# mlefkir/Pioran.jl

Hardware: AMD Instinct MI355X
Metric: logpdf evals/sec (batched) at N=1e4, J=20; max |Δlogℒ| vs reference (higher is better)
Workload: dtype f64; 1 GPU; N=10000 irregular series, SHO-20 (J=20 celerite terms, R=40 active rows), batch=4096 draws per GPU, shared (c,d), per-draw mu/nu; inputs HBM-resident; N=10000, J=20, R_active=40, batch_per_gpu=4096, global_batch=4096, kernel_config=tile, parallelism=batch-sharded x1, all-gather of logL

## Files before the change

pioran.jl_amd/csrc/celerite_tile.hip:

```cpp
#include "common.h"
#include "window_common.h"

#ifndef PIORAN_TSTAMP
#define PIORAN_TSTAMP(i) __builtin_amdgcn_sched_barrier(0)
#define PIORAN_TSTAMP_DECL
#define PIORAN_TSTAMP_FLUSH
#endif
#ifndef PIORAN_ASTAMP2
#define PIORAN_ASTAMP2(i) __builtin_amdgcn_sched_barrier(0)
#define PIORAN_ASTAMP2_DECL
#define PIORAN_ASTAMP2_FLUSH
#endif

namespace {

constexpr int kTileMaxTerms = 64;
constexpr int kTileWaves = 4;
#define PIORAN_LDS_ORDER() asm volatile("" ::: "memory")
template <int NB, bool CD = false>
constexpr int tile_adj_waves() { return NB <= 3 ? 4 : (CD ? 2 : 3); }

template <int NB>
struct TileWave {
    double scr[16 * 18];
    double2 albe[16 * NB];
    double ck[16 * NB + 16];
    double ys[16];
    double up[NB > 1 ? NB * (NB - 1) / 2 : 1][16 * 18];
};

constexpr int kPairWin = 5;
template <int JQ>
__global__ void __launch_bounds__(256) tile_pairs_mfma_kernel(const ScanParams p, const double* __restrict__ btab, int64_t rsb, int64_t tsp, double* __restrict__ out)
{
    const int J = p.J;
    const int64_t NW = (p.N + KW - 1) / KW;
    const int lane = threadIdx.x & 63, w = threadIdx.x >> 6, li = lane & 15, lk = lane >> 4;
    const int64_t b0 = ((int64_t)blockIdx.y * 4 + w) * 16;
    if (b0 >= p.B) return;
    const int64_t draw = b0 + li < p.B ? b0 + li : p.B - 1;
    double aop[JQ], bop[JQ];
    int toff[JQ];
#pragma unroll
    for (int q = 0; q < JQ; ++q) {
        const int t = 4 * q + lk;
        aop[q] = t < J ? p.A[draw * J + t] : 0.0;
        bop[q] = t < J ? p.Bc[draw * J + t] : 0.0;
        toff[q] = (t < J ? t : J - 1) * 128 + 4 * (li & 3) + (li >> 2);
    }
    const bool live = b0 + li < p.B;
    double* orow = out + (b0 + li) * NW * 128 + 4 * lk;
    const int64_t k0 = (int64_t)blockIdx.x * kPairWin, k1 = k0 + kPairWin < NW ? k0 + kPairWin : NW;
    for (int64_t k = k0; k < k1; ++k) {
        const double2* E = reinterpret_cast<const double2*>(btab + k * rsb + tsp);
#pragma unroll 2
        for (int pt = 0; pt < 8; ++pt) {
            double2 e[JQ];
#pragma unroll
            for (int q = 0; q < JQ; ++q) e[q] = E[toff[q] + 16 * pt];
            d4 acc = {0.0, 0.0, 0.0, 0.0};
#pragma unroll
            for (int q = 0; q < JQ; ++q) {
                acc = __builtin_amdgcn_mfma_f64_16x16x4f64(e[q].x, aop[q], acc, 0, 0, 0);
                acc = __builtin_amdgcn_mfma_f64_16x16x4f64(e[q].y, bop[q], acc, 0, 0, 0);
            }
            if (live) *reinterpret_cast<d4*>(orow + k * 128 + 16 * pt) = acc;
        }
    }
}

template <typename... Args>
static inline bool launch_pairs_mfma(const ScanParams& p, hipStream_t stream, Args... args)
{
    const int64_t NW = (p.N + KW - 1) / KW;
    if ((p.B + 63) / 64 > 65535 || p.J > kTileMaxTerms) return false;
    const dim3 gr((unsigned)((NW + kPairWin - 1) / kPairWin), (unsigned)((p.B + 63) / 64));
    const int jq = (p.J + 3) / 4;
    if (jq <= 5) hipLaunchKernelGGL(tile_pairs_mfma_kernel<5>, gr, dim3(256), 0, stream, p, args...);
    else if (jq <= 10) hipLaunchKernelGGL(tile_pairs_mfma_kernel<10>, gr, dim3(256), 0, stream, p, args...);
    else if (jq <= 16) hipLaunchKernelGGL(tile_pairs_mfma_kernel<16>, gr, dim3(256), 0, stream, p, args...);
    else return false;
    return true;
}

template <int NB, int KL = 4, bool ST = false, bool SER = false>
__global__ void __launch_bounds__(64 * kTileWaves, NB <= 4 ? 2 : 1) celerite_tile_kernel(const ScanParams p, const double* __restrict__ btab,
                                                                                          const double* __restrict__ pairs)
{
    constexpr int TS = 3 * NB * 256 + 16 * NB + 16, TSP = (TS + 127) & ~127;
    static_assert(!(ST && SER), "the gradient's forward pass takes the shared series only");
    extern __shared__ double lds_[];
    const int tid = threadIdx.x;
    const int w = __builtin_amdgcn_readfirstlane(tid >> 6);
    const int lane = tid & 63, q = lane >> 4, c16 = lane & 15;
    const int64_t b = (int64_t)blockIdx.x * kTileWaves + w;
    if (b >= p.B) return;
    const int64_t N = p.N;
    const int J = p.J, R = p.R;
    const int64_t NW = (N + KW - 1) / KW;
    const int64_t RSB = TSP + 256 * (int64_t)J;
    TileWave<NB>& sw = reinterpret_cast<TileWave<NB>*>(lds_)[w];
    const __amdgpu_buffer_rsrc_t rs_tab = __builtin_amdgcn_make_buffer_rsrc(const_cast<double*>(btab), 0, 0x7ffffffc, 0x00020000);
    const __amdgpu_buffer_rsrc_t rs_pw = __builtin_amdgcn_make_buffer_rsrc(const_cast<double*>(pairs + b * NW * 128), 0, 0x7ffffffc, 0x00020000);
    const int lane8 = lane * 8;
    const int rsb8 = (int)(RSB * 8);
    constexpr int Jy = NB - 1;
    const int ry = R & 15;
    const double mu = p.mu ? p.mu[b] : 0.0;
    const double nu = p.nu ? p.nu[b] : 1.0;
    const bool has_nu = p.nu != nullptr;
    const double* __restrict__ Ab_ = p.A + b * J;
    const double* __restrict__ Bb_ = p.Bc + b * J;
    double suma = 0.0;
    for (int j = 0; j < J; ++j) suma += Ab_[j];

    for (int r = lane; r < 16 * NB; r += 64) {
        double a = 0.0, bb = 0.0;
        if (r < R) {
            const int rm = p.rowmap[r];
            const int term = rm & 0xfffff;
            a = Ab_[term];
            bb = ((rm >> 30) & 1) ? -Bb_[term] : Bb_[term];
        }
        sw.albe[r] = double2{a, bb};
    }
    constexpr int NU = NB * (NB - 1) / 2;
    for (int i = lane; i < (NU > 0 ? NU : 1) * 16 * 18; i += 64) (&sw.up[0][0])[i] = 0.0;
    asm volatile("s_waitcnt lgkmcnt(0)" ::: "memory");

    constexpr int NT = NB * (NB + 1) / 2;
    auto tix = [](int I, int Jc) constexpr { return I * (I + 1) / 2 + Jc; };
    auto uix = [](int I, int Jc) constexpr { return I * (I - 1) / 2 + Jc; };
    d4 T[NT];
#pragma unroll
    for (int i = 0; i < NT; ++i) T[i] = d4{0.0, 0.0, 0.0, 0.0};
    double Uf[NB][4];

    double cvn[4], cxn[4];
    auto live_k = [](int I, int ks) constexpr { return I < NB - 1 || ks < KL; };
    auto fetch_u = [&](int64_t k, int I) __attribute__((always_inline)) {
        const int so = (int)k * rsb8;
#pragma unroll
        for (int ks = 0; ks < 4; ++ks) {
            if (!live_k(I, ks)) continue;
            cvn[ks] = buf_load_f64(rs_tab, lane8, so + (I * 4 + ks) * 512);
            cxn[ks] = buf_load_f64(rs_tab, lane8, so + (NB * 256 + (I * 4 + ks) * 64) * 8);
        }
    };
    auto form_u = [&](int I) __attribute__((always_inline)) {
        if (I == NB - 1 && KL == 0) return;
        double2 cf[4];
#pragma unroll
        for (int ks = 0; ks < 4; ++ks)
            if (live_k(I, ks)) cf[ks] = sw.albe[16 * I + 4 * ks + q];
        asm volatile("s_waitcnt lgkmcnt(0)" ::: "memory");
#pragma unroll
        for (int ks = 0; ks < 4; ++ks)
            if (live_k(I, ks)) Uf[I][ks] = fma(cf[ks].x, cvn[ks], cf[ks].y * cxn[ks]);
    };
    constexpr int NCK = (16 * NB + 16 + 63) / 64;
    double ckpre[NCK];
    auto fetch_ck = [&](int64_t k) __attribute__((always_inline)) {
        const int so = (int)k * rsb8 + 3 * NB * 256 * 8;
#pragma unroll
        for (int i = 0; i < NCK; ++i) ckpre[i] = buf_load_f64(rs_tab, lane8, so + 512 * i);
    };
    int pidx[4];
#pragma unroll
    for (int g = 0; g < 4; ++g) {
        const int r = 4 * g + q, hi = r > c16 ? r : c16, lo = r > c16 ? c16 : r;
        pidx[g] = 8 * (r == c16 ? 127 : hi * (hi - 1) / 2 + lo);
    }
    const int gd = (c16 - q) >> 2;
    const bool on_diag = ((c16 - q) & 3) == 0;
    double apre[4];
    auto fetch_A = [&](int64_t k) __attribute__((always_inline)) {
#pragma unroll
        for (int g = 0; g < 4; ++g) apre[g] = buf_load_f64(rs_pw, pidx[g], (int)k * 1024);
    };
    [[maybe_unused]] double ypre = 0.0, spre = 0.0;
    auto fetch_series = [&](int64_t k) __attribute__((always_inline)) {
        if constexpr (SER) {
            int64_t n = k * KW + c16;
            n = n < N ? n : N - 1;
            ypre = p.Y[b * N + n];
            spre = p.S2[b * N + n];
        }
    };
    fetch_A(0);
    fetch_ck(0);
    fetch_series(0);
#pragma unroll
    for (int I = 0; I < NB; ++I) {
        fetch_u(0, I);
        form_u(I);
    }
    const double mu_y = c16 == ry ? mu : 0.0;
    const int64_t k_ragged = (N % KW) ? NW - 1 : NW;
    double quad = 0.0;
    double Pm = 1.0;
    int Pe = 0;
    bool nonpd = false;

    PIORAN_TSTAMP_DECL
    for (int64_t k = 0; k < NW; ++k) {
        PIORAN_TSTAMP(0);
        const int wso = (int)k * rsb8;
        const bool more = k + 1 < NW;
#pragma unroll
        for (int i = 0; i < NCK; ++i)
            if (lane + 64 * i < 16 * NB + 16) sw.ck[lane + 64 * i] = ckpre[i];
        if constexpr (SER) {
            asm volatile("s_waitcnt lgkmcnt(0)" ::: "memory");
            if (lane < 16) { sw.ys[lane] = ypre; sw.ck[16 * NB + lane] = spre; }
        }
        if (more) { fetch_ck(k + 1); fetch_series(k + 1); }
        if constexpr (ST) {
            d4* gtk = reinterpret_cast<d4*>(p.gw + ((b * NW + k) * NT) * 256);
#pragma unroll
            for (int i = 0; i < NT; ++i) gtk[i * 64 + lane] = T[i];
        }
        constexpr bool VHA = NB <= 3 || NB >= 5;
        [[maybe_unused]] double vha[VHA ? NB : 1][4];
        if constexpr (VHA) {
#pragma unroll
            for (int I = 0; I < NB; ++I)
#pragma unroll
                for (int g = 0; g < 4; ++g) vha[I][g] = buf_load_f64(rs_tab, lane8, wso + (2 * NB * 256 + (I * 4 + g) * 64) * 8);
            if (k == k_ragged) {
#pragma unroll
                for (int I = 0; I < NB; ++I)
#pragma unroll
                    for (int g = 0; g < 4; ++g)
                        if (k * KW + 4 * g + q >= N) vha[I][g] = I == Jy ? mu_y : 0.0;
            }
        }
        d4 x[NB];
#pragma unroll
        for (int Jc = 0; Jc < NB; ++Jc) {
            d4 acc = {0.0, 0.0, 0.0, 0.0};
#pragma unroll
            for (int I = 0; I < Jc; ++I) {
                double bt[4];
#pragma unroll
                for (int ks = 0; ks < 4; ++ks) bt[ks] = sw.up[uix(Jc, I)][c16 * 18 + 4 * ks + q];
#pragma unroll
                for (int ks = 0; ks < 4; ++ks) acc = __builtin_amdgcn_mfma_f64_16x16x4f64(Uf[I][ks], bt[ks], acc, 0, 0, 0);
            }
#pragma unroll
            for (int I = Jc; I < NB; ++I)
#pragma unroll
                for (int ks = 0; ks < 4; ++ks)
                    if (live_k(I, ks)) acc = __builtin_amdgcn_mfma_f64_16x16x4f64(Uf[I][ks], T[tix(I, Jc)][ks], acc, 0, 0, 0);
            x[Jc] = acc;
        }
        PIORAN_TSTAMP(1);
        d4 G = {0.0, 0.0, 0.0, 0.0};
        double vh[4];
        if constexpr (!VHA) {
#pragma unroll
            for (int g = 0; g < 4; ++g) vh[g] = buf_load_f64(rs_tab, lane8, wso + (2 * NB * 256 + g * 64) * 8);
        }
        [[maybe_unused]] double ysv[4] = {0.0, 0.0, 0.0, 0.0};
        if constexpr (SER) {
#pragma unroll
            for (int g = 0; g < 4; ++g) ysv[g] = sw.ys[4 * g + q];
        }
#pragma unroll
        for (int Jc = 0; Jc < NB; ++Jc) {
            const bool gk = Jc < NB - 1 || KL > 0;
            if (gk) {
#pragma unroll
                for (int g = 0; g < 4; ++g) sw.scr[(4 * g + q) * 18 + c16] = x[Jc][g];
            }
            PIORAN_LDS_ORDER();
            double mb[4];
#pragma unroll
            for (int ks = 0; ks < 4; ++ks)
                if (live_k(Jc, ks)) mb[ks] = sw.scr[c16 * 18 + 4 * ks + q];
            const double ckc = sw.ck[16 * Jc + c16];
            asm volatile("s_waitcnt lgkmcnt(0)" ::: "memory");
#pragma unroll
            for (int ks = 0; ks < 4; ++ks)
                if (live_k(Jc, ks)) G = __builtin_amdgcn_mfma_f64_16x16x4f64(Uf[Jc][ks], mb[ks], G, 0, 0, 0);
#pragma unroll
            for (int g = 0; g < 4; ++g) {
                double v;
                if constexpr (VHA) v = vha[Jc][g]; else v = vh[g];
                if (Jc == Jy) v -= mu_y;
                x[Jc][g] = fma(-ckc, x[Jc][g], v);
                asm volatile("" : "+v"(x[Jc][g]));
            }
            if constexpr (!VHA) {
                if (Jc + 1 < NB) {
#pragma unroll
                    for (int g = 0; g < 4; ++g) vh[g] = buf_load_f64(rs_tab, lane8, wso + (2 * NB * 256 + ((Jc + 1) * 4 + g) * 64) * 8);
                }
            }
            __builtin_amdgcn_sched_barrier(0);
        }
        if constexpr (!VHA) {
            if (k == k_ragged) {
#pragma unroll
                for (int Jc = 0; Jc < NB; ++Jc)
#pragma unroll
                    for (int g = 0; g < 4; ++g) {
                        const double vt = buf_load_f64(rs_tab, lane8, wso + (2 * NB * 256 + (Jc * 4 + g) * 64) * 8);
                        if (k * KW + 4 * g + q >= N) x[Jc][g] -= Jc == Jy ? vt - mu_y : vt;
                    }
            }
        }
        if constexpr (SER) {
#pragma unroll
            for (int g = 0; g < 4; ++g) {
                double vt;
                if constexpr (VHA) vt = vha[Jy][g]; else vt = buf_load_f64(rs_tab, lane8, wso + (2 * NB * 256 + (Jy * 4 + g) * 64) * 8);
                const bool pad = k == k_ragged && k * KW + 4 * g + q >= N;
                if (c16 == ry && !pad) x[Jy][g] += ysv[g] - vt;
            }
        }
        PIORAN_TSTAMP(2);
        PIORAN_TSTAMP(3);
        {
            const double s2n = sw.ck[16 * NB + c16];
            const double dg = k * KW + c16 < N ? suma + (has_nu ? nu * s2n : s2n) : 1.0;
#pragma unroll
            for (int g = 0; g < 4; ++g) sw.scr[(4 * g + q) * 16 + c16] = ((on_diag && g == gd) ? dg : apre[g]) - G[g];
        }
        if (k + 1 < NW) fetch_A(k + 1);
        PIORAN_LDS_ORDER();
        double m[16];
#pragma unroll
        for (int j = 0; j < 16; ++j) m[j] = sw.scr[j * 16 + c16];
        asm volatile("s_waitcnt lgkmcnt(0)" ::: "memory");
        PIORAN_TSTAMP(4);
        __builtin_amdgcn_s_setprio(2);
        double mult = ldl_first_mult(m, c16);
        static_for<0, 16>([&](auto Pc) __attribute__((always_inline)) { ldl_step<decltype(Pc)::value>(m, mult, c16); });
        __builtin_amdgcn_s_setprio(0);
        PIORAN_TSTAMP(5);
        if (q == 0) {
            double2* dst = reinterpret_cast<double2*>(sw.scr + c16 * 18);
#pragma unroll
            for (int j = 0; j < 16; j += 2) dst[j / 2] = double2{m[j], m[j + 1]};
        }
        PIORAN_LDS_ORDER();
        double li[4], idv[4];
#pragma unroll
        for (int ks = 0; ks < 4; ++ks) {
            const int kk = 4 * ks + q;
            const double lv = sw.scr[kk * 18 + c16];
            idv[ks] = recip_f64(sw.scr[kk * 18 + kk]);
            li[ks] = kk < c16 ? lv * idv[ks] : (kk == c16 ? 1.0 : 0.0);
        }
        {
            const double dj = sw.scr[c16 * 18 + c16];
            nonpd |= !(dj > 0.0);
            Pm *= (k == 0 && c16 == 0) ? dj : fabs(dj);
            int ex;
            Pm = frexp(Pm, &ex);
            Pe += ex;
        }
        asm volatile("s_waitcnt lgkmcnt(0)" ::: "memory");
        PIORAN_TSTAMP(6);
        if (more) fetch_u(k + 1, 0);
        __builtin_amdgcn_sched_barrier(0);
        d4 yt[NB];
#pragma unroll
        for (int Jc = 0; Jc < NB; ++Jc) {
            d4 a = {0.0, 0.0, 0.0, 0.0};
#pragma unroll
            for (int ks = 0; ks < 4; ++ks) a = __builtin_amdgcn_mfma_f64_16x16x4f64(li[ks], x[Jc][ks], a, 0, 0, 0);
            yt[Jc] = a;
        }
        PIORAN_TSTAMP(7);
        constexpr bool CKP = NB <= 3 || NB >= 5;
        [[maybe_unused]] double ckrow[CKP ? NB : 1][4], ckcol[CKP ? NB : 1];
        if constexpr (CKP) {
#pragma unroll
            for (int I = 0; I < NB; ++I) {
#pragma unroll
                for (int g = 0; g < 4; ++g) ckrow[I][g] = sw.ck[16 * I + 4 * g + q];
                ckcol[I] = sw.ck[16 * I + c16];
            }
        }
        auto ck_row = [&](int I, int g) __attribute__((always_inline)) -> double { if constexpr (CKP) return ckrow[I][g]; else return sw.ck[16 * I + 4 * g + q]; };
#pragma unroll
        for (int Jc = 0; Jc < NB; ++Jc) {
            if (more) {
                form_u(Jc);
                if (Jc + 1 < NB) fetch_u(k + 1, Jc + 1);
            }
            double ysc[4];
            double ckc;
            if constexpr (CKP) ckc = ckcol[Jc]; else ckc = sw.ck[16 * Jc + c16];
#pragma unroll
            for (int g = 0; g < 4; ++g) {
                ysc[g] = yt[Jc][g] * idv[g];
                if (Jc == Jy) quad = fma(yt[Jc][g], ysc[g], quad);
            }
#pragma unroll
            for (int I = Jc; I < NB; ++I) {
#pragma unroll
                for (int g = 0; g < 4; ++g) T[tix(I, Jc)][g] *= ck_row(I, g) * ckc;
#pragma unroll
                for (int ks = 0; ks < 4; ++ks) T[tix(I, Jc)] = __builtin_amdgcn_mfma_f64_16x16x4f64(yt[I][ks], ysc[ks], T[tix(I, Jc)], 0, 0, 0);
                if (Jc < I) {
#pragma unroll
                    for (int g = 0; g < 4; ++g) sw.up[uix(I, Jc)][(4 * g + q) * 18 + c16] = T[tix(I, Jc)][g];
                }
            }
            __builtin_amdgcn_sched_barrier(0);
        }
        PIORAN_TSTAMP(8);
        PIORAN_LDS_ORDER();
    }

    PIORAN_TSTAMP_FLUSH
    asm volatile("s_waitcnt lgkmcnt(0)" ::: "memory");
    if (c16 == ry) sw.scr[q] = quad;
    if (q == 0) sw.scr[16 + c16] = log(Pm) + (double)Pe * 0.6931471805599453094;
    const bool any_nonpd = __builtin_amdgcn_ballot_w64(nonpd) != 0;
    asm volatile("s_waitcnt lgkmcnt(0)" ::: "memory");
    if (lane == 0) {
        const double qs = (sw.scr[0] + sw.scr[1]) + (sw.scr[2] + sw.scr[3]);
        double logdet = 0.0;
        for (int j = 0; j < 16; ++j) logdet += sw.scr[16 + j];
        const double res = -0.5 * logdet - 0.5 * (double)N * 1.8378770664093454836 - 0.5 * qs;
        p.out[b] = res;
        if (p.status) p.status[b] = !isfinite(res) ? 2 : (any_nonpd ? 1 : 0);
    }
}

template <int NB, bool CD = false>
struct TileAdjWave {
    double scr[16 * 18];
    double srm[16 * 16];
    double2 albe[16 * NB];
    double ck[16 * NB + 16];
    double qy[16];
    double red[16 * NB][4];
    double tk[NB * (NB + 1) / 2][16 * 18];
    double upB[NB > 1 ? NB * (NB - 1) / 2 : 1][16 * 18];
    double mw[CD ? NB : 1][CD ? 256 : 1];
    double accd[CD ? 2 * NB : 1][CD ? 64 : 1];
    double tm[CD ? 24 : 1];
    double scrb[(NB <= 3 && !CD) ? NB : 1][(NB <= 3 && !CD) ? 16 * 18 : 1];
    double acab[2 * NB][64];
};

template <int NB, bool CD>
constexpr bool tile_adj_batched() { return NB <= 3 && !CD; }
template <int NB, bool CD = false>
__global__ void __launch_bounds__((64 * tile_adj_waves<NB, CD>()), 1) celerite_tile_adjoint_kernel(const ScanParams p, const double* __restrict__ btab,
                                                                                                  const double* __restrict__ gtab, double* __restrict__ pairs,
                                                                                                  double* __restrict__ grad_a, double* __restrict__ grad_b,
                                                                                                  double* __restrict__ grad_nu, double* __restrict__ grad_mu,
                                                                                                  double* __restrict__ grad_c, double* __restrict__ grad_d)
{
    constexpr int TS = 3 * NB * 256 + 16 * NB + 16, TSP = (TS + 127) & ~127;
    constexpr int64_t GS = 4 * (int64_t)NB * 256 + 16 * NB + 16 + 24;
    constexpr int NT = NB * (NB + 1) / 2, NU = NB * (NB - 1) / 2;
    constexpr bool BT = tile_adj_batched<NB, CD>();
    extern __shared__ double lds_[];
    const int tid = threadIdx.x;
    const int w = __builtin_amdgcn_readfirstlane(tid >> 6);
    const int lane = tid & 63, q = lane >> 4, c16 = lane & 15;
    const int64_t b = (int64_t)blockIdx.x * tile_adj_waves<NB, CD>() + w;
    if (b >= p.B) return;
    const int64_t N = p.N;
    const int J = p.J, R = p.R;
    const int64_t NW = (N + KW - 1) / KW;
    const int64_t RSB = TSP + 256 * (int64_t)J;
    TileAdjWave<NB, CD>& sw = reinterpret_cast<TileAdjWave<NB, CD>*>(lds_)[w];
    const __amdgpu_buffer_rsrc_t rs_tab = __builtin_amdgcn_make_buffer_rsrc(const_cast<double*>(btab), 0, 0x7ffffffc, 0x00020000);
    const __amdgpu_buffer_rsrc_t rs_gt = __builtin_amdgcn_make_buffer_rsrc(const_cast<double*>(gtab), 0, 0x7ffffffc, 0x00020000);
    double* const pw = pairs + b * NW * 128;
    const double* const gtb = p.gw + b * NW * NT * 256;
    const int lane8 = lane * 8;
    const int rsb8 = (int)(RSB * 8), gs8 = (int)(GS * 8);
    constexpr int Jy = NB - 1;
    const int ry = R & 15;
    const double mu = p.mu ? p.mu[b] : 0.0;
    const double nu = p.nu ? p.nu[b] : 1.0;
    const bool has_nu = p.nu != nullptr;
    const double* __restrict__ Ab_ = p.A + b * J;
    const double* __restrict__ Bb_ = p.Bc + b * J;
    double suma = 0.0;
    for (int j = 0; j < J; ++j) suma += Ab_[j];
    for (int r = lane; r < 16 * NB; r += 64) {
        double a = 0.0, bb = 0.0;
        if (r < R) {
            const int rm = p.rowmap[r];
            const int term = rm & 0xfffff;
            a = Ab_[term];
            bb = ((rm >> 30) & 1) ? -Bb_[term] : Bb_[term];
        }
        sw.albe[r] = double2{a, bb};
    }
    for (int i = lane; i < (NU > 0 ? NU : 1) * 16 * 18; i += 64) (&sw.upB[0][0])[i] = 0.0;
    asm volatile("s_waitcnt lgkmcnt(0)" ::: "memory");
    double2 myab[NB];
    double ymask[NB], mu_sel[NB];
#pragma unroll
    for (int Jc = 0; Jc < NB; ++Jc) {
        myab[Jc] = sw.albe[16 * Jc + c16];
        ymask[Jc] = (Jc == Jy && c16 == ry) ? 1.0 : 0.0;
        mu_sel[Jc] = ymask[Jc] * mu;
    }
    auto tix = [](int I, int Jc) constexpr { return I * (I + 1) / 2 + Jc; };
    auto uix = [](int I, int Jc) constexpr { return I * (I - 1) / 2 + Jc; };
    d4 Tb[NT];
#pragma unroll
    for (int i = 0; i < NT; ++i) Tb[i] = d4{0.0, 0.0, 0.0, 0.0};
#pragma unroll
    for (int Jc = 0; Jc < 2 * NB; ++Jc) sw.acab[Jc][lane] = 0.0;
    double acc_mu = 0.0, acc_sa = 0.0, acc_nu = 0.0;
    if constexpr (CD) {
#pragma unroll
        for (int Jc = 0; Jc < 2 * NB; ++Jc) sw.accd[Jc][lane] = 0.0;
    }
    auto lds_add = [](double* slot, double v) __attribute__((always_inline)) {
        if constexpr (CD) *slot += v;
        else (void)__hip_atomic_fetch_add(slot, v, __ATOMIC_RELAXED, __HIP_MEMORY_SCOPE_WAVEFRONT);
    };
    [[maybe_unused]] auto add_c = [&](int Jc, double v) __attribute__((always_inline)) { lds_add(&sw.accd[Jc][lane], v); };
    [[maybe_unused]] auto add_d = [&](int Jc, double v) __attribute__((always_inline)) { lds_add(&sw.accd[NB + Jc][lane], v); };
    [[maybe_unused]] constexpr int OFF_H = 2 * NB * 256 + 16 * NB + 16, OFF_TM = OFF_H + 2 * NB * 256;
    int pidx[4];
#pragma unroll
    for (int g = 0; g < 4; ++g) {
        const int r = 4 * g + q, hi = r > c16 ? r : c16, lo = r > c16 ? c16 : r;
        pidx[g] = r == c16 ? 127 : hi * (hi - 1) / 2 + lo;
    }
    const int gd = (c16 - q) >> 2;
    const bool on_diag = ((c16 - q) & 3) == 0;
    int pnn[2], pjj[2];
#pragma unroll
    for (int h = 0; h < 2; ++h) {
        const int pq = lane + 64 * h;
        int n_ = 1;
        while ((n_ + 1) * n_ / 2 <= pq) ++n_;
        pnn[h] = n_ < 16 ? n_ : 15;
        pjj[h] = n_ < 16 ? pq - n_ * (n_ - 1) / 2 : 0;
    }
    const int64_t k_ragged = (N % KW) ? NW - 1 : NW;
    constexpr int NCK = (16 * NB + 16 + 63) / 64;
    constexpr int NWARM = (NT * 2048 + 8191) / 8192;
    constexpr bool PFT = NB <= 3;
    struct WinIn {
        d4 T[PFT ? NT : 1];
        double cva[PFT ? NB : 1][4], cxa[PFT ? NB : 1][4];
        double ckp[NCK];
        double ap[4];
        float warm[PFT ? 1 : NWARM];
    };
    auto fetch_win = [&](int64_t kk, WinIn& wi) __attribute__((always_inline)) {
        const int wso = (int)kk * rsb8;
        const d4* tk = reinterpret_cast<const d4*>(gtb + kk * NT * 256);
        if constexpr (PFT) {
#pragma unroll
            for (int i = 0; i < NT; ++i) wi.T[i] = tk[i * 64 + lane];
        } else {
            const float* tw = reinterpret_cast<const float*>(tk);
#pragma unroll
            for (int j = 0; j < NWARM; ++j) {
                const int line = j * 64 + lane;
                wi.warm[j] = tw[(line < NT * 16 ? line : NT * 16 - 1) * 32];
            }
        }
        if constexpr (PFT) {
#pragma unroll
            for (int I = 0; I < NB; ++I)
#pragma unroll
                for (int ks = 0; ks < 4; ++ks) {
                    wi.cva[I][ks] = buf_load_f64(rs_tab, lane8, wso + (I * 4 + ks) * 512);
                    wi.cxa[I][ks] = buf_load_f64(rs_tab, lane8, wso + (NB * 256 + (I * 4 + ks) * 64) * 8);
                }
        }
#pragma unroll
        for (int i = 0; i < NCK; ++i) wi.ckp[i] = buf_load_f64(rs_tab, lane8, wso + 3 * NB * 256 * 8 + 512 * i);
#pragma unroll
        for (int g = 0; g < 4; ++g) wi.ap[g] = pw[kk * 128 + pidx[g]];
    };
    WinIn cur;
    fetch_win(NW - 1, cur);
    PIORAN_ASTAMP2_DECL

    for (int64_t k = NW - 1; k >= 0; --k) {
        PIORAN_ASTAMP2(0);
        const int wso = (int)k * rsb8, gso = (int)k * gs8;
        [[maybe_unused]] d4 tnow[PFT ? 1 : NT];
        [[maybe_unused]] double cvh[PFT ? 1 : NB][4], cxh[PFT ? 1 : NB][4];
        if constexpr (!PFT) {
#pragma unroll
            for (int j = 0; j < NWARM; ++j) asm volatile("" ::"v"(cur.warm[j]));
#pragma unroll
            for (int I = 0; I < NB; ++I)
#pragma unroll
                for (int ks = 0; ks < 4; ++ks) {
                    cvh[I][ks] = buf_load_f64(rs_tab, lane8, wso + (I * 4 + ks) * 512);
                    cxh[I][ks] = buf_load_f64(rs_tab, lane8, wso + (NB * 256 + (I * 4 + ks) * 64) * 8);
                }
            const d4* tkg = reinterpret_cast<const d4*>(gtb + k * NT * 256);
#pragma unroll
            for (int i = 0; i < NT; ++i) tnow[i] = tkg[i * 64 + lane];
            __builtin_amdgcn_sched_barrier(0);
        }
        double vhs[NB][4];
#pragma unroll
        for (int I = 0; I < NB; ++I)
#pragma unroll
            for (int g = 0; g < 4; ++g) vhs[I][g] = buf_load_f64(rs_tab, lane8, wso + (2 * NB * 256 + (I * 4 + g) * 64) * 8);
        if (k == k_ragged) {
#pragma unroll
            for (int I = 0; I < NB; ++I)
#pragma unroll
                for (int g = 0; g < 4; ++g)
                    if (k * KW + 4 * g + q >= N) vhs[I][g] = mu_sel[I];
        }
#pragma unroll
        for (int i = 0; i < NCK; ++i)
            if (lane + 64 * i < 16 * NB + 16) sw.ck[lane + 64 * i] = cur.ckp[i];
        double apre[4];
#pragma unroll
        for (int g = 0; g < 4; ++g) apre[g] = cur.ap[g];
        double Uf[NB][4];
#pragma unroll
        for (int I = 0; I < NB; ++I)
#pragma unroll
            for (int ks = 0; ks < 4; ++ks) {
                const double2 cf = sw.albe[16 * I + 4 * ks + q];
                if constexpr (PFT) Uf[I][ks] = fma(cf.x, cur.cva[I][ks], cf.y * cur.cxa[I][ks]);
                else Uf[I][ks] = fma(cf.x, cvh[I][ks], cf.y * cxh[I][ks]);
            }
        if constexpr (PFT) {
#pragma unroll
            for (int i = 0; i < NT; ++i)
#pragma unroll
                for (int g = 0; g < 4; ++g) sw.tk[i][(4 * g + q) * 18 + c16] = cur.T[i][g];
        } else {
#pragma unroll
            for (int i = 0; i < NT; ++i)
#pragma unroll
                for (int g = 0; g < 4; ++g) sw.tk[i][(4 * g + q) * 18 + c16] = tnow[i][g];
        }
        PIORAN_LDS_ORDER();
        __builtin_amdgcn_sched_barrier(0);
        PIORAN_ASTAMP2(1);
        d4 x[NB];
#pragma unroll
        for (int Jc = 0; Jc < NB; ++Jc) {
            d4 acc = {0.0, 0.0, 0.0, 0.0};
#pragma unroll
            for (int I = 0; I < Jc; ++I) {
                double bt[4];
#pragma unroll
                for (int ks = 0; ks < 4; ++ks) bt[ks] = sw.tk[tix(Jc, I)][c16 * 18 + 4 * ks + q];
#pragma unroll
                for (int ks = 0; ks < 4; ++ks) acc = __builtin_amdgcn_mfma_f64_16x16x4f64(Uf[I][ks], bt[ks], acc, 0, 0, 0);
            }
#pragma unroll
            for (int I = Jc; I < NB; ++I) {
                double bt[4];
#pragma unroll
                for (int ks = 0; ks < 4; ++ks) bt[ks] = sw.tk[tix(I, Jc)][(4 * ks + q) * 18 + c16];
#pragma unroll
                for (int ks = 0; ks < 4; ++ks) acc = __builtin_amdgcn_mfma_f64_16x16x4f64(Uf[I][ks], bt[ks], acc, 0, 0, 0);
            }
            x[Jc] = acc;
        }
        __builtin_amdgcn_sched_barrier(0);
        PIORAN_ASTAMP2(2);
        d4 G = {0.0, 0.0, 0.0, 0.0};
        if constexpr (BT) {
            double mb[NB][4], ckc[NB];
#pragma unroll
            for (int Jc = 0; Jc < NB; ++Jc)
#pragma unroll
                for (int g = 0; g < 4; ++g) sw.scrb[Jc][(4 * g + q) * 18 + c16] = x[Jc][g];
            PIORAN_LDS_ORDER();
#pragma unroll
            for (int Jc = 0; Jc < NB; ++Jc) {
#pragma unroll
                for (int ks = 0; ks < 4; ++ks) mb[Jc][ks] = sw.scrb[Jc][c16 * 18 + 4 * ks + q];
                ckc[Jc] = sw.ck[16 * Jc + c16];
            }
            asm volatile("s_waitcnt lgkmcnt(0)" ::: "memory");
#pragma unroll
            for (int Jc = 0; Jc < NB; ++Jc)
#pragma unroll
                for (int ks = 0; ks < 4; ++ks) G = __builtin_amdgcn_mfma_f64_16x16x4f64(Uf[Jc][ks], mb[Jc][ks], G, 0, 0, 0);
#pragma unroll
            for (int Jc = 0; Jc < NB; ++Jc)
#pragma unroll
                for (int g = 0; g < 4; ++g) {
                    double v = vhs[Jc][g] - mu_sel[Jc];
                    x[Jc][g] = fma(-ckc[Jc], x[Jc][g], v);
                    asm volatile("" : "+v"(x[Jc][g]));
                }
        } else {
#pragma unroll
        for (int Jc = 0; Jc < NB; ++Jc) {
#pragma unroll
            for (int g = 0; g < 4; ++g) sw.scr[(4 * g + q) * 18 + c16] = x[Jc][g];
            if constexpr (CD) {
#pragma unroll
// ... 721 lines not shown
```

Baseline: 449,100 evals/s.

## Hoist T-tile ck rescaling into LDL latency slots and share pivot reciprocals

For small NB, the per-tile ck row/column rescaling of the T accumulators moves out of the MFMA update loop. It is interleaved into earlier points: the last row block is rescaled before the LDL factorization and the others after the pivot reads, so the VALU work can overlap LDS waits. Pivot reciprocals are now computed once per column, written to LDS, and read back, replacing four recip_f64 calls per lane. The fetch_u prefetch is also issued earlier. This adds register pressure from the extra ck arrays and asm barriers, and depends on LDS ordering for the shared reciprocals.

```diff
diff --git a/pioran.jl_amd/csrc/celerite_tile.hip b/pioran.jl_amd/csrc/celerite_tile.hip
--- a/pioran.jl_amd/csrc/celerite_tile.hip
+++ b/pioran.jl_amd/csrc/celerite_tile.hip
@@ -202,6 +202,16 @@
     int Pe = 0;
     bool nonpd = false;
 
+    constexpr bool PRE = NB <= 3;
+    [[maybe_unused]] double ckl[4], ckcl[NB], cku[NB > 1 ? NB - 1 : 1][4];
+    [[maybe_unused]] auto rescale_tile = [&](int I, int Jc, const double (&row)[4]) __attribute__((always_inline)) {
+#pragma unroll
+        for (int g = 0; g < 4; ++g) {
+            T[tix(I, Jc)][g] *= row[g] * ckcl[Jc];
+            if (!(KL == 0 && I == NB - 1 && Jc == NB - 1)) asm volatile("" : "+v"(T[tix(I, Jc)][g]));
+        }
+    };
+
     PIORAN_TSTAMP_DECL
     for (int64_t k = 0; k < NW; ++k) {
         PIORAN_TSTAMP(0);
@@ -321,6 +331,12 @@
         }
         PIORAN_TSTAMP(2);
         PIORAN_TSTAMP(3);
+        if constexpr (PRE) {
+#pragma unroll
+            for (int g = 0; g < 4; ++g) ckl[g] = sw.ck[16 * (NB - 1) + 4 * g + q];
+#pragma unroll
+            for (int Jc = 0; Jc < NB; ++Jc) ckcl[Jc] = sw.ck[16 * Jc + c16];
+        }
         {
             const double s2n = sw.ck[16 * NB + c16];
             const double dg = k * KW + c16 < N ? suma + (has_nu ? nu * s2n : s2n) : 1.0;
@@ -332,6 +348,12 @@
         double m[16];
 #pragma unroll
         for (int j = 0; j < 16; ++j) m[j] = sw.scr[j * 16 + c16];
+        if constexpr (PRE) {
+            __builtin_amdgcn_sched_barrier(0);
+#pragma unroll
+            for (int Jc = 0; Jc < NB; ++Jc) rescale_tile(NB - 1, Jc, ckl);
+            __builtin_amdgcn_sched_barrier(0);
+        }
         asm volatile("s_waitcnt lgkmcnt(0)" ::: "memory");
         PIORAN_TSTAMP(4);
         __builtin_amdgcn_s_setprio(2);
@@ -346,24 +368,41 @@
         }
         PIORAN_LDS_ORDER();
         double li[4], idv[4];
+        const double dj = sw.scr[c16 * 18 + c16];
+        double lv[4];
+#pragma unroll
+        for (int ks = 0; ks < 4; ++ks) lv[ks] = sw.scr[(4 * ks + q) * 18 + c16];
+        if constexpr (PRE) {
+#pragma unroll
+            for (int I = 0; I < NB - 1; ++I)
+#pragma unroll
+                for (int g = 0; g < 4; ++g) cku[I][g] = sw.ck[16 * I + 4 * g + q];
+        }
+        if (more) fetch_u(k + 1, 0);
+        const double rj = recip_f64(dj);
+        if (q == 0) sw.scr[c16 * 18 + 16] = rj;
+        PIORAN_LDS_ORDER();
+#pragma unroll
+        for (int ks = 0; ks < 4; ++ks) idv[ks] = sw.scr[(4 * ks + q) * 18 + 16];
+        nonpd |= !(dj > 0.0);
+        Pm *= (k == 0 && c16 == 0) ? dj : fabs(dj);
+        int ex;
+        Pm = frexp(Pm, &ex);
+        Pe += ex;
+        if constexpr (PRE && NB > 1) {
+            __builtin_amdgcn_sched_barrier(0);
+#pragma unroll
+            for (int Jc = 0; Jc < NB - 1; ++Jc)
+#pragma unroll
+                for (int I = Jc; I < NB - 1; ++I) rescale_tile(I, Jc, cku[I]);
+            __builtin_amdgcn_sched_barrier(0);
+        }
 #pragma unroll
         for (int ks = 0; ks < 4; ++ks) {
             const int kk = 4 * ks + q;
-            const double lv = sw.scr[kk * 18 + c16];
-            idv[ks] = recip_f64(sw.scr[kk * 18 + kk]);
-            li[ks] = kk < c16 ? lv * idv[ks] : (kk == c16 ? 1.0 : 0.0);
-        }
-        {
-            const double dj = sw.scr[c16 * 18 + c16];
-            nonpd |= !(dj > 0.0);
-            Pm *= (k == 0 && c16 == 0) ? dj : fabs(dj);
-            int ex;
-            Pm = frexp(Pm, &ex);
-            Pe += ex;
-        }
-        asm volatile("s_waitcnt lgkmcnt(0)" ::: "memory");
+            li[ks] = kk < c16 ? lv[ks] * idv[ks] : (kk == c16 ? 1.0 : 0.0);
+        }
         PIORAN_TSTAMP(6);
-        if (more) fetch_u(k + 1, 0);
         __builtin_amdgcn_sched_barrier(0);
         d4 yt[NB];
 #pragma unroll
@@ -374,7 +413,7 @@
             yt[Jc] = a;
         }
         PIORAN_TSTAMP(7);
-        constexpr bool CKP = NB <= 3 || NB >= 5;
+        constexpr bool CKP = NB >= 5;
         [[maybe_unused]] double ckrow[CKP ? NB : 1][4], ckcol[CKP ? NB : 1];
         if constexpr (CKP) {
 #pragma unroll
@@ -384,7 +423,7 @@
                 ckcol[I] = sw.ck[16 * I + c16];
             }
         }
-        auto ck_row = [&](int I, int g) __attribute__((always_inline)) -> double { if constexpr (CKP) return ckrow[I][g]; else return sw.ck[16 * I + 4 * g + q]; };
+        [[maybe_unused]] auto ck_row = [&](int I, int g) __attribute__((always_inline)) -> double { if constexpr (CKP) return ckrow[I][g]; else return sw.ck[16 * I + 4 * g + q]; };
 #pragma unroll
         for (int Jc = 0; Jc < NB; ++Jc) {
             if (more) {
@@ -392,8 +431,8 @@
                 if (Jc + 1 < NB) fetch_u(k + 1, Jc + 1);
             }
             double ysc[4];
-            double ckc;
-            if constexpr (CKP) ckc = ckcol[Jc]; else ckc = sw.ck[16 * Jc + c16];
+            [[maybe_unused]] double ckc = 0.0;
+            if constexpr (CKP) ckc = ckcol[Jc]; else if constexpr (!PRE) ckc = sw.ck[16 * Jc + c16];
 #pragma unroll
             for (int g = 0; g < 4; ++g) {
                 ysc[g] = yt[Jc][g] * idv[g];
@@ -401,8 +440,10 @@
             }
 #pragma unroll
             for (int I = Jc; I < NB; ++I) {
-#pragma unroll
-                for (int g = 0; g < 4; ++g) T[tix(I, Jc)][g] *= ck_row(I, g) * ckc;
+                if constexpr (!PRE) {
+#pragma unroll
+                    for (int g = 0; g < 4; ++g) T[tix(I, Jc)][g] *= ck_row(I, g) * ckc;
+                }
 #pragma unroll
                 for (int ks = 0; ks < 4; ++ks) T[tix(I, Jc)] = __builtin_amdgcn_mfma_f64_16x16x4f64(yt[I][ks], ysc[ks], T[tix(I, Jc)], 0, 0, 0);
                 if (Jc < I) {
```

After: 459,500 evals/s, median of 6. 1.02x the previous value.
